# clearmatics/libff

Hardware: AMD Instinct MI355X
Metric: G1 MSM throughput (scalar-muls/sec) (higher is better)
Workload: dtype u32

## Files before the change

### libff_amd/csrc/msm_group.hip

```cpp
#include "curve_params.h"
#include "ec.cuh"
#include "fp2h.cuh"
#include "group_vtable.h"
#include "wide.cuh"
#include "wide28.cuh"
#include "rr.cuh"

#include <algorithm>
#include <cstdio>
#include <vector>
#include <type_traits>

#ifndef AMDMSM_GROUP
#error "compile with -DAMDMSM_GROUP=<group traits> -DAMDMSM_VT=<vtable getter name>"
#endif

namespace amdmsm {
template <bool I>
struct ec_coeff_a<Fp<AMDMSM_GROUP::fq, I>> {
    static constexpr int value = AMDMSM_GROUP::DEG == 1 ? AMDMSM_GROUP::COEFF_A : 0;
};
template <int NR, bool I>
struct ec_coeff_a<Fp2<AMDMSM_GROUP::fq, NR, I>> {
    static constexpr int value = AMDMSM_GROUP::DEG == 2 ? AMDMSM_GROUP::COEFF_A : 0;
// ... 1925 lines not shown
AMDMSM_DEV typename std::enable_if<(P::N >= 16 && P::N < 32), void>::type horner_chain(
    Jac<Fp<P, I>>& res, const uint32_t* __restrict__ window_sums, int W, int c, const uint32_t* __restrict__ init) {
    using F = WideFq<P>;
    const WideEnv<P> env = wide_env<P>();
    auto load = [&](const uint32_t* p, uint32_t& X, uint32_t& Y, uint32_t& Z) {
        X = env.valid ? p[env.j] : 0u;
        Y = env.valid ? p[EW + env.j] : 0u;
        Z = env.valid ? p[2 * EW + env.j] : 0u;
    };
    uint32_t X, Y, Z, X2, Y2, Z2;
    int w = W - 1;
    if (init) {
        load(init, X, Y, Z);
    } else {
        load(window_sums + (size_t)w * XYZW, X, Y, Z);
        --w;
    }
    for (; w >= 0; --w) {
        if (!wide_is_zero(Z)) {
            if (c >= 4) jac_dbl_run28<P>(env, X, Y, Z, c);
            else for (int i = 0; i < c; ++i) jac_dbl_wide2<P>(env, X, Y, Z);
        }
        load(window_sums + (size_t)w * XYZW, X2, Y2, Z2);
        jac_add_seq<F, P>(env, X, Y, Z, X2, Y2, Z2);
    }
    wide_to_packed(res.x, X);
    wide_to_packed(res.y, Y);
    wide_to_packed(res.z, Z);
}
template <class P, int NR, bool I>
AMDMSM_DEV typename std::enable_if<(P::N < 16), void>::type horner_chain(Jac<Fp2<P, NR, I>>& res,
                                                                         const uint32_t* __restrict__ window_sums, int W,
                                                                         int c, const uint32_t* __restrict__ init) {
    using F = WideFq2<P, NR>;
    const WideEnv<P> env = wide_env<P>();
    const uint32_t wi = F::word_index(env);
    auto load = [&](const uint32_t* p, uint32_t& X, uint32_t& Y, uint32_t& Z) {
        X = env.valid ? p[wi] : 0u;
        Y = env.valid ? p[EW + wi] : 0u;
        Z = env.valid ? p[2 * EW + wi] : 0u;
    };
    uint32_t X, Y, Z, X2, Y2, Z2;
    int w = W - 1;
    if (init) {
        load(init, X, Y, Z);
    } else {
        load(window_sums + (size_t)w * XYZW, X, Y, Z);
        --w;
    }
    for (; w >= 0; --w) {
        if (!wide_is_zero(Z)) {
            if constexpr (GP::COEFF_A != 0) for (int i = 0; i < c; ++i) jac_dbl_seq<F, P, GP::COEFF_A>(env, X, Y, Z);
            else if (c >= 4) jac_dbl_run28q<P, NR>(env, X, Y, Z, c);
            else for (int i = 0; i < c; ++i) jac_dbl_seq<F, P>(env, X, Y, Z);
        }
        load(window_sums + (size_t)w * XYZW, X2, Y2, Z2);
        jac_add_seq<F, P, GP::COEFF_A>(env, X, Y, Z, X2, Y2, Z2);
    }
    wide_to_packed(res.x.c0, from_row(X, 0));
    wide_to_packed(res.x.c1, from_row(X, 1));
    wide_to_packed(res.y.c0, from_row(Y, 0));
    wide_to_packed(res.y.c1, from_row(Y, 1));
    wide_to_packed(res.z.c0, from_row(Z, 0));
    wide_to_packed(res.z.c1, from_row(Z, 1));
}
template <class EE>
AMDMSM_DEV void horner_chain(Jac<EE>& res, const uint32_t* __restrict__ window_sums, int W, int c,
                             const uint32_t* __restrict__ init, ...) {
    Jac<EE> x;
    int w = W - 1;
    if (init) {
        load_jac(res, init);
    } else {
        load_jac(res, window_sums + (size_t)w * XYZW);
        --w;
    }
    for (; w >= 0; --w) {
        for (int i = 0; i < c; ++i) jac_dbl_lanes3(res);
        load_jac(x, window_sums + (size_t)w * XYZW);
        jac_add(res, res, x);
    }
}

__global__ void __launch_bounds__(64) k_horner(const uint32_t* __restrict__ window_sums, int W, int c, int form,
                                               const uint32_t* __restrict__ init, uint32_t* __restrict__ out) {
    __builtin_amdgcn_s_setprio(3);
    Jac<E> res;
    horner_chain(res, window_sums, W, c, init);
    if (threadIdx.x == 0) store_out(out, res, form);
}

constexpr int WH_MAX_GROUPS = 6;
__global__ void __launch_bounds__(64 * WH_MAX_GROUPS) k_window_horner(const uint32_t* __restrict__ planes, int c,
                                                                       uint32_t* __restrict__ out) {
    __shared__ uint32_t grp[WH_MAX_GROUPS * XYZW];
    __builtin_amdgcn_s_setprio(3);
    const int wave = (int)(threadIdx.x >> 6), ng = (c + 3) / 4;
    Jac<E> res;
    if (wave < ng) {
        const int k0 = 4 * wave, cnt = (c - k0 < 4) ? c - k0 : 4;
        horner_chain(res, planes + ((size_t)blockIdx.x * c + k0) * XYZW, cnt, 1, nullptr);
        if ((threadIdx.x & 63u) == 0) store_jac(grp + wave * XYZW, res);
    }
    __syncthreads();
    if (wave != 0) return;
    horner_chain(res, grp, ng, 4, nullptr);
    if (threadIdx.x == 0) store_jac(out + (size_t)blockIdx.x * XYZW, res);
}

struct horner_outs {
    uint32_t* p[8];
};
__global__ void __launch_bounds__(64) k_horner_batch(const uint32_t* __restrict__ window_sums, int W, int c, int form,
                                                     horner_outs outs) {
    __builtin_amdgcn_s_setprio(3);
    Jac<E> res;
    horner_chain(res, window_sums + (size_t)blockIdx.x * W * XYZW, W, c, nullptr);
    uint32_t* out = outs.p[0];
#pragma unroll
    for (int j = 1; j < 8; ++j) out = (blockIdx.x == (unsigned)j) ? outs.p[j] : out;
    if (threadIdx.x == 0) store_out(out, res, form);
}

__global__ void __launch_bounds__(64) k_sum_points(const uint32_t* __restrict__ pts, int k, int form,
                                                   uint32_t* __restrict__ out) {
    Jac<E> res;
    if (k <= 0) jac_set_inf(res);
    else horner_chain(res, pts, k, 0, nullptr);
    if (threadIdx.x == 0) store_out(out, res, form);
}

constexpr int IMPORT_K = 32;

__global__ void __launch_bounds__(TPB) k_import_bases(const uint32_t* __restrict__ src, size_t stride_words,
                                                      int form_special, size_t n, uint32_t* __restrict__ dst) {
    if (form_special) {
        const size_t i = gtid();
        if (i >= n) return;
        const uint32_t* q = src + i * stride_words;
        Aff<E> a;
        E z;
        el_load(a.x, q);
        el_load(a.y, q + EW);
        el_load(z, q + 2 * EW);
        if (el_is_zero(z)) {
            el_zero(a.x);
            el_zero(a.y);
        }
        store_aff(dst + i * AFFW, a);
        return;
    }
    const size_t i0 = gtid() * IMPORT_K;
    if (i0 >= n) return;
    const size_t i1 = (i0 + IMPORT_K < n) ? i0 + IMPORT_K : n;
    E one, acc;
    el_one(one);
    acc = one;
    bool trivial = true;
    for (size_t i = i0; i < i1; ++i) {
        Jac<E> p;
        load_libff(p, src + i * stride_words);
        if (jac_is_inf(p)) continue;
        el_store(dst + i * AFFW, acc);
        if (!el_eq(p.z, one)) {
            trivial = false;
            el_mul(acc, acc, p.z);
        }
    }
    E inv = one;
    if (!trivial) el_inv(inv, acc);
    for (size_t i = i1; i-- > i0;) {
        Jac<E> p;
        load_libff(p, src + i * stride_words);
        Aff<E> a;
        if (jac_is_inf(p)) {
            el_zero(a.x);
            el_zero(a.y);
        } else if (el_eq(p.z, one)) {
            a.x = p.x;
            a.y = p.y;
        } else {
            E pre, zi, z2;
            el_load(pre, dst + i * AFFW);
            el_mul(zi, inv, pre);
            el_mul(inv, inv, p.z);
            el_sqr(z2, zi);
            el_mul(a.x, p.x, z2);
            el_mul(z2, z2, zi);
            el_mul(a.y, p.y, z2);
        }
        store_aff(dst + i * AFFW, a);
    }
}

__global__ void __launch_bounds__(TPB) k_export_affine(const uint32_t* __restrict__ src, size_t n,
                                                       uint32_t* __restrict__ dst) {
    const size_t i = gtid();
    if (i >= n) return;
    Aff<E> a;
    load_aff(a, src + i * AFFW);
// ... 884 lines not shown
#pragma unroll
        for (int j = FRW - 1; j >= 0; --j) rec[j] = (rec[j] << SMV_W) | (j ? rec[j - 1] >> (32 - SMV_W) : 0u);
        const bool neg = (f >> (SMV_W - 1)) != 0;
        const uint32_t mag = neg ? (1u << SMV_W) - f : f;
        if (mag) {
            load_aff(e, table + ((size_t)(mag - 1) * n + i) * AFFW);
            el_cneg(e.y, e.y, neg);
            xyzz_madd(acc, e);
        }
    }
    Jac<E> res;
    xyzz_to_jac(res, acc);
    store_out(out + i * XYZW, res, form);
}

constexpr int SEG_DS = (SMV_DIGITS + 3) / 4 * 4;

__global__ void __launch_bounds__(TPB) k_seg_digits(const uint32_t* __restrict__ scalars, size_t n, int mont,
                                                    uint32_t* __restrict__ digits) {
    const size_t i = gtid();
    if (i >= n) return;
    uint32_t s[FRW];
    load_scalar(s, scalars, i, mont);
    uint32_t* row = digits + i * (SEG_DS / 4);
    uint32_t word = 0;
    for_each_signed_digit(s, SMV_W, SMV_DIGITS, [&](int w, int32_t d) {
        word |= ((uint32_t)d & 0xffu) << ((w & 3) * 8);
        if ((w & 3) == 3 || w == SMV_DIGITS - 1) {
            row[w >> 2] = word;
            word = 0;
        }
    });
}

__global__ void __launch_bounds__(TPB) k_seg_accumulate(const uint32_t* __restrict__ table, size_t nt,
                                                        const signed char* __restrict__ digits,
                                                        const uint4* __restrict__ slices, size_t lanes,
                                                        uint32_t* __restrict__ sums) {
    const size_t lane = gtid();
    if (lane >= lanes) return;
    const size_t sl = lane / SMV_DIGITS;
    const uint32_t w = (uint32_t)(lane - sl * SMV_DIGITS);
    const uint4 s = slices[sl];
    Xyzz<E> acc;
    xyzz_set_inf(acc);
    Aff<E> e;
    const signed char* dp = digits + (size_t)s.x * SEG_DS + w;
    size_t col = s.z;
#pragma unroll 1
    for (uint32_t t = s.x; t < s.y; ++t, ++col, dp += SEG_DS) {
        const int d = *dp;
        if (d) {
            const uint32_t mag = (uint32_t)(d < 0 ? -d : d);
            load_aff(e, table + ((size_t)(mag - 1) * nt + col) * AFFW);
            el_cneg(e.y, e.y, d < 0);
            xyzz_madd(acc, e);
        }
    }
    store_xyzz(sums + lane * ZZW, acc);
}

__global__ void __launch_bounds__(TPB) k_seg_fold(const uint32_t* __restrict__ sums, const uint32_t* __restrict__ seg_first,
                                                  size_t lanes, uint32_t* __restrict__ winsum) {
    const size_t lane = gtid();
    if (lane >= lanes) return;
    const size_t seg = lane / SMV_DIGITS;
    const uint32_t w = (uint32_t)(lane - seg * SMV_DIGITS);
    Xyzz<E> acc, x;
    xyzz_set_inf(acc);
#pragma unroll 1
    for (uint32_t sl = seg_first[seg]; sl < seg_first[seg + 1]; ++sl) {
        load_xyzz(x, sums + ((size_t)sl * SMV_DIGITS + w) * ZZW);
        xyzz_add(acc, acc, x);
    }
    Jac<E> r;
    xyzz_to_jac(r, acc);
    store_jac(winsum + lane * XYZW, r);
}

__global__ void __launch_bounds__(64) k_seg_horner(const uint32_t* __restrict__ winsum, int form, uint32_t* __restrict__ out) {
    Jac<E> res;
    horner_chain(res, winsum + (size_t)blockIdx.x * SMV_DIGITS * XYZW, SMV_DIGITS, SMV_W, nullptr);
    if (threadIdx.x == 0) store_out(out + (size_t)blockIdx.x * XYZW, res, form);
}

constexpr int FOLD_DS = (SMV_DIGITS + 3) / 4 * 4;
static_assert(2 * FOLD_MAX_K * FOLD_DS <= (int)FOLD_DIGIT_BYTES, "the digit rows fit the buffer the engine sets aside");
struct alignas(16) fold_scalars {
    uint32_t w[FOLD_MAX_K * FRW];
};

__global__ void __launch_bounds__(64) k_fold_digits(const fold_scalars sc, int k, int mont, int glv, int W,
                                                    uint32_t* __restrict__ digits) {
    const int j = (int)threadIdx.x;
    if (j >= k) return;
    uint32_t s[FRW];
    load_scalar(s, sc.w, (size_t)j, mont);
    uint32_t word = 0;
    auto put = [&](int row, int w, int32_t d) {
        word |= ((uint32_t)d & 0xffu) << ((w & 3) * 8);
        if ((w & 3) == 3 || w == W - 1) {
            digits[row * (FOLD_DS / 4) + (w >> 2)] = word;
            word = 0;
        }
    };
    if (glv) {
        if constexpr (GP::HAS_ENDO) for_each_glv_digit(s, SMV_W, W, [&](int h, int w, int32_t d) { put(2 * j + h, w, d); });
    } else {
        for_each_signed_digit(s, SMV_W, W, [&](int w, int32_t d) { put(j, w, d); });
    }
}

__global__ void __launch_bounds__(TPB) k_fold_ladder(const uint32_t* __restrict__ tables, size_t n,
                                                     const uint32_t* __restrict__ digits, int rows, int glv, int W,
                                                     int form, uint32_t* __restrict__ out) {
    const size_t i = gtid();
    if (i >= n) return;
    int top = -1;
#pragma unroll 1
    for (int q = (W + 3) / 4 - 1; q >= 0 && top < 0; --q) {
        uint32_t any = 0;
#pragma unroll 1
        for (int r = 0; r < rows; ++r) any |= digits[r * (FOLD_DS / 4) + q];
        if (any) top = 4 * q + (31 - __clz((int)any)) / 8;
    }
    const signed char* dg = (const signed char*)digits;
    Xyzz<E> acc;
    xyzz_set_inf(acc);
    Aff<E> e;
#pragma unroll 1
    for (int w = top; w >= 0; --w) {
        if (w != top) {
#pragma unroll 1
            for (int b = 0; b < SMV_W; ++b) xyzz_dbl(acc, acc);
        }
#pragma unroll 1
        for (int r = 0; r < rows; ++r) {
            const int d = dg[r * FOLD_DS + w];
            if (d) {
                const uint32_t mag = (uint32_t)(d < 0 ? -d : d);
                const size_t t = (size_t)(glv ? r >> 1 : r);
                load_aff(e, tables + ((t * SMV_T + (mag - 1)) * n + i) * AFFW);
                if constexpr (GP::HAS_ENDO) {
                    if (glv && (r & 1)) scale_by_beta(e.x);
                }
                el_cneg(e.y, e.y, d < 0);
                xyzz_madd(acc, e);
            }
        }
    }
    Jac<E> res;
    xyzz_to_jac(res, acc);
    store_out(out + i * XYZW, res, form);
}

inline unsigned blocks_for(size_t n, int tpb = TPB) { return (unsigned)((n + tpb - 1) / tpb); }

void l_import_bases(hipStream_t st, const uint32_t* src, size_t stride_words, int form_special, size_t n, uint32_t* dst) {
    if (!n) return;
    const size_t lanes = form_special ? n : (n + IMPORT_K - 1) / IMPORT_K;
    hipLaunchKernelGGL(k_import_bases, dim3(blocks_for(lanes)), dim3(TPB), 0, st, src, stride_words, form_special, n, dst);
}
void l_precompute_table(hipStream_t st, const uint32_t* bases, size_t n, int c, int D, uint32_t* tmp, uint32_t* table) {
    if (!n) return;
    hipLaunchKernelGGL(k_precompute_table, dim3(blocks_for(n)), dim3(TPB), 0, st, bases, n, c, D, tmp, table);
}
// ... 179 lines not shown
                fwrite(h.data(), 8, h.size(), f);
                fclose(f);
            }
        }
    }
#else
    hipLaunchKernelGGL(k_accumulate, dim3(blocks_for((size_t)W * T * ACC_LANES)), dim3(TPB), dyn_lds, st, ends, lists,
                       list_stride, bases, buckets, part_first, part_last, cont_bucket, W, B, S, T, endo_pts,
                       endo_pts ? (uint32_t)n_real : 0x80000000u, sync_waves);
#endif
}
void l_endo_points(hipStream_t st, const uint32_t* bases, size_t n, uint32_t* out) {
    if (!n) return;
    hipLaunchKernelGGL(k_endo_points, dim3(blocks_for(n * 2 * GP::DEG)), dim3(TPB), 0, st, bases, n, out);
}
void l_glv_digits(hipStream_t st, const uint32_t* scalars, size_t n, int mont, int c, int W, int32_t* out) {
    if (!n) return;
    hipLaunchKernelGGL(k_glv_digits, dim3(blocks_for(n)), dim3(TPB), 0, st, scalars, n, mont, c, W, out);
}
size_t l_accumulate_resident_lanes(int overlap) {
    auto query = [](size_t dyn_lds) {
        int dev = 0, cus = 256, blocks = 0;
        if (hipGetDevice(&dev) == hipSuccess) (void)hipDeviceGetAttribute(&cus, hipDeviceAttributeMultiprocessorCount, dev);
        if (hipOccupancyMaxActiveBlocksPerMultiprocessor(&blocks, k_accumulate, TPB, dyn_lds) != hipSuccess || blocks <= 0) blocks = 4;
        return (size_t)cus * (size_t)blocks * TPB / ACC_LANES;
    };
    static const size_t lanes = query(0);
    static const size_t lanes_overlap = (AMDMSM_OVERLAP_OK && ACC_OVERLAP_LDS) ? query(ACC_OVERLAP_LDS) : lanes;
    return overlap ? lanes_overlap : lanes;
}
void l_accumulate_fixup(hipStream_t st, const uint32_t* ends, uint32_t* buckets, uint32_t* part_first,
                        const uint32_t* part_last, const uint32_t* cont_bucket, uint32_t* queue, int W, uint32_t B,
                        uint32_t S, uint32_t T) {
    const unsigned fix_blocks = blocks_for((size_t)W * T * RED_LANES, 64);
    const unsigned compact_blocks = T / FIX_BLOCK >= 2 ? (unsigned)(W * (T / FIX_BLOCK - 1)) : 0u;
    hipLaunchKernelGGL(k_accumulate_fixup, dim3(fix_blocks + compact_blocks), dim3(64), 0, st, ends, part_first,
                       part_last, cont_bucket, buckets, queue, W, B, S, T, fix_blocks);
    const size_t lanes = (size_t)W * T;
    const size_t cap_mid = fixup_queue_cap_mid(lanes) / (RED_FOLD / MID_G) + 1, cap_long = fixup_queue_cap_long(lanes);
    const unsigned mid_blocks = (unsigned)(cap_mid < 8192 ? cap_mid : 8192), long_blocks = (unsigned)(cap_long < 2048 ? cap_long : 2048);
    hipLaunchKernelGGL(k_accumulate_fixup_queue, dim3(mid_blocks + long_blocks), dim3(64), 0, st, ends,
                       part_first, part_last, cont_bucket, buckets, queue, mid_blocks, lanes, B, S, T);
}
void l_reduce_segments(hipStream_t st, const uint32_t* buckets, int W, uint32_t B, uint32_t L, uint32_t* out) {
    hipLaunchKernelGGL(k_reduce_segments, dim3(blocks_for((size_t)W * (B / L) * RED_LANES, 64)), dim3(64), 0, st, buckets, W, B,
                       L, out);
}
void l_sum_butterfly(hipStream_t st, const uint32_t* in, int W, uint32_t M, uint32_t* out) {
    hipLaunchKernelGGL(k_sum_butterfly, dim3(blocks_for((size_t)W * M * RED_LANES, 64)), dim3(64), 0, st, in, W, M, out);
}
void l_sum_block(hipStream_t st, const uint32_t* in, int W, uint32_t M, uint32_t* out) {
    if (M >= 8 && M * RED_LANES <= (uint32_t)SUMW_THREADS && (M & (M - 1)) == 0) {
        hipLaunchKernelGGL(k_sum_block_wide, dim3(W), dim3(SUMW_THREADS), 0, st, in, W, M, out);
        return;
    }
    const unsigned threads = (unsigned)((M * RED_LANES + 63) / 64 * 64);
    hipLaunchKernelGGL(k_sum_block, dim3(W), dim3(threads), 0, st, in, W, M, out);
}
void l_reduce_rowcol(hipStream_t st, const uint32_t* buckets, int W, uint32_t B, int c, uint32_t q_row, uint32_t q_col,
                     uint32_t* rc, uint32_t* planes, uint32_t* out) {
    const int h = c / 2;
    const uint32_t C = 1u << h, R = B >> h;
    auto fit = [](uint32_t len, uint32_t q) {
        if (q < 1) q = 1;
        while (q & (q - 1)) q &= q - 1;
        if (q > len) q = len;
        while (len / q > RED_FOLD) q <<= 1;
        return q;
    };
    q_row = fit(C, q_row);
    q_col = fit(R, q_col);
    const size_t row_lanes = (size_t)W * (R + 1) * (C / q_row) * RED_LANES, col_lanes = (size_t)W * C * (R / q_col) * RED_LANES;
    const unsigned row_blocks = blocks_for(row_lanes, 64), col_blocks = blocks_for(col_lanes, 64);
    hipLaunchKernelGGL(k_bucket_sums, dim3(row_blocks + col_blocks), dim3(64), 0, st, buckets, W, B, h, q_row, q_col, row_blocks, rc);
    const uint32_t maxm = (C > R ? C : R) / 2;
    static const bool wide_planes = !(getenv("AMDMSM_PLANES_WIDE") && atoi(getenv("AMDMSM_PLANES_WIDE")) == 0);
    if (maxm >= 8 && wide_planes) {
        hipLaunchKernelGGL(k_plane_sums_wide, dim3((unsigned)(W * c)), dim3(SUMW_THREADS), 0, st, rc, W, c, h, planes);
    } else {
        unsigned threads = (unsigned)((maxm * RED_LANES + 63) / 64 * 64);
        threads = threads < 64 ? 64 : (threads > 256 ? 256 : threads);
        hipLaunchKernelGGL(k_plane_sums, dim3((unsigned)(W * c)), dim3(threads), 0, st, rc, W, c, h, planes);
    }
    hipLaunchKernelGGL(k_window_horner, dim3((unsigned)W), dim3((unsigned)(64 * ((c + 3) / 4))), 0, st, planes, c, out);
}
void l_horner(hipStream_t st, const uint32_t* window_sums, int W, int c, int form, const uint32_t* init, uint32_t* out) {
    hipLaunchKernelGGL(k_horner, dim3(1), dim3(64), 0, st, window_sums, W, c, form, init, out);
}
void l_horner_batch(hipStream_t st, const uint32_t* window_sums, int k, int W, int c, int form, uint32_t* const* outs) {
    horner_outs o = {};
    for (int j = 0; j < k && j < 8; ++j) o.p[j] = outs[j];
    hipLaunchKernelGGL(k_horner_batch, dim3((unsigned)k), dim3(64), 0, st, window_sums, W, c, form, o);
}
void l_sum_points(hipStream_t st, const uint32_t* pts, int k, int form, uint32_t* out) {
    hipLaunchKernelGGL(k_sum_points, dim3(1), dim3(64), 0, st, pts, k, form, out);
}
void l_gen_bases_seq(hipStream_t st, unsigned long long first, size_t n, uint32_t* dst) {
    if (!n) return;
    hipLaunchKernelGGL(k_gen_bases_seq, dim3(blocks_for(n)), dim3(TPB), 0, st, first, n, dst);
}
void l_export_affine(hipStream_t st, const uint32_t* src, size_t n, uint32_t* dst) {
    if (!n) return;
    hipLaunchKernelGGL(k_export_affine, dim3(blocks_for(n)), dim3(TPB), 0, st, src, n, dst);
}
void l_ffi_decode_points(hipStream_t st, const uint32_t* src, size_t n, uint32_t* dst, uint32_t* status) {
    if (!n) return;
    hipLaunchKernelGGL(k_ffi_decode_points, dim3(blocks_for(n)), dim3(TPB), 0, st, src, n, dst, status);
}
void l_ffi_decode_scalars(hipStream_t st, const uint32_t* src, size_t n, uint32_t* dst, uint32_t* status) {
    if (!n) return;
    hipLaunchKernelGGL(k_ffi_decode_scalars, dim3(blocks_for(n)), dim3(TPB), 0, st, src, n, dst, status);
}
void l_ffi_encode_point(hipStream_t st, const uint32_t* src_xyz, uint32_t* dst) {
    hipLaunchKernelGGL(k_ffi_encode_point, dim3(1), dim3(64), 0, st, src_xyz, dst);
}
void l_disk_decode(hipStream_t st, const uint32_t* src, size_t n, uint32_t* dst) {
    if (!n) return;
    hipLaunchKernelGGL(k_disk_decode, dim3(blocks_for(n)), dim3(TPB), 0, st, src, n, dst);
}
void l_disk_decode_compressed(hipStream_t st, const uint32_t* src, size_t n, uint32_t* dst, uint32_t* status) {
    if (!n) return;
    hipLaunchKernelGGL(k_disk_decode_compressed, dim3(blocks_for(n, 64)), dim3(64), 0, st, src, n, dst, status);
}
#if AMDMSM_ACC_RR
template <class G>
bool launch_fb_exp_rr(hipStream_t st, const uint32_t* table_aff, const uint32_t* scalars, size_t n, int mont, const uint32_t* coeff,
                      int scalar_size, int window, int form, uint32_t* out) {
    if constexpr (G::DEG == 1) {
        if (window < 32) {
            hipLaunchKernelGGL(k_fb_exp_rr<G>, dim3(blocks_for(n)), dim3(TPB), 0, st, table_aff, scalars, n, mont, coeff, scalar_size,
                               window, form, out);
            return true;
        }
    }
    return false;
}
#endif
void l_fixed_base_exp(hipStream_t st, const uint32_t* g_xyz, int scalar_size, int window, const uint32_t* scalars, size_t n,
                      int mont, const uint32_t* coeff, int form, uint32_t* gouter, uint32_t* table, uint32_t* table_aff,
                      int build_table, uint32_t* out) {
    const int outerc = (scalar_size + window - 1) / window;
    if (build_table) {
        hipLaunchKernelGGL(k_fb_gouter, dim3(1), dim3(64), 0, st, g_xyz, outerc, window, gouter);
        for (int level = 0; level < window; ++level) {
            const size_t per_level = level == 0 ? 2 : ((size_t)1 << level);
            hipLaunchKernelGGL(k_fb_table_level, dim3(blocks_for((size_t)outerc * per_level)), dim3(TPB), 0, st, gouter, outerc,
                               window, scalar_size, level, table);
        }
        const size_t entries = (size_t)outerc << window;
        hipLaunchKernelGGL(k_fb_table_affine, dim3(blocks_for((entries + FB_NORM_K - 1) / FB_NORM_K)), dim3(TPB), 0, st, table,
                           entries, table_aff);
    }
    if (n) {
#if AMDMSM_ACC_RR
        if (launch_fb_exp_rr<GP>(st, table_aff, scalars, n, mont, coeff, scalar_size, window, form, out)) return;
#endif
        hipLaunchKernelGGL(k_fb_exp, dim3(blocks_for(n)), dim3(TPB), 0, st, table_aff, scalars, n, mont, coeff, scalar_size,
                           window, form, out);
    }
}
void l_field_op(hipStream_t st, int op, const uint32_t* a, const uint32_t* b, uint32_t* out, size_t n) {
    if (!n) return;
    hipLaunchKernelGGL(k_field_op, dim3(blocks_for(n)), dim3(TPB), 0, st, op, a, b, out, n);
}
void l_field_probe(hipStream_t st, int impl, int op, const uint32_t* a, const uint32_t* b, const uint32_t* c, const uint32_t* d,
                   uint32_t* out, uint32_t* flag, size_t n) {
    if (!n) return;
    if (impl) hipLaunchKernelGGL(k_field_probe<EI>, dim3(blocks_for(n)), dim3(TPB), 0, st, op, a, b, c, d, out, flag, n);
    else hipLaunchKernelGGL(k_field_probe<E>, dim3(blocks_for(n)), dim3(TPB), 0, st, op, a, b, c, d, out, flag, n);
}
void l_xyzz_probe(hipStream_t st, int impl, int op, const uint32_t* acc, const uint32_t* pt, uint32_t* out, size_t n) {
    if (!n) return;
    if (impl) hipLaunchKernelGGL(k_xyzz_probe<EI>, dim3(blocks_for(n)), dim3(TPB), 0, st, op, acc, pt, out, n);
    else hipLaunchKernelGGL(k_xyzz_probe<E>, dim3(blocks_for(n)), dim3(TPB), 0, st, op, acc, pt, out, n);
}
void l_group_op(hipStream_t st, int op, const uint32_t* a, const uint32_t* b, uint32_t* out, size_t n, int form) {
    if (!n) return;
    hipLaunchKernelGGL(k_group_op, dim3(blocks_for(n)), dim3(TPB), 0, st, op, a, b, out, n, form);
}
void l_digits(hipStream_t st, const uint32_t* scalars, size_t n, int mont, int c, int W, int32_t* out) {
    if (!n) return;
    hipLaunchKernelGGL(k_digits, dim3(blocks_for(n)), dim3(TPB), 0, st, scalars, n, mont, c, W, out);
}
void l_mul_bench(hipStream_t st, uint32_t* inout, size_t nthreads, int iters, int inline_variant) {
    if (!nthreads) return;
#if AMDMSM_BENCH_BOTH
    if (inline_variant) {
        hipLaunchKernelGGL(k_mul_bench<true>, dim3(blocks_for(nthreads)), dim3(TPB), 0, st, inout, nthreads, iters);
        return;
    }
#endif
    hipLaunchKernelGGL(k_mul_bench<false>, dim3(blocks_for(nthreads)), dim3(TPB), 0, st, inout, nthreads, iters);
}
void l_madd_bench(hipStream_t st, const uint32_t* pts, uint32_t* out, size_t nthreads, int iters, int inline_variant) {
    if (!nthreads) return;
    if (inline_variant == 2) {
        hipLaunchKernelGGL(k_xyzz_madd_bench<EH>, dim3(blocks_for(nthreads)), dim3(TPB), 0, st, pts, out, nthreads, iters);
        return;
    }
#if AMDMSM_BENCH_BOTH
    if (inline_variant) {
        hipLaunchKernelGGL(k_madd_bench<EI>, dim3(blocks_for(nthreads)), dim3(TPB), 0, st, pts, out, nthreads, iters);
        return;
    }
#endif
    hipLaunchKernelGGL(k_madd_bench<E>, dim3(blocks_for(nthreads)), dim3(TPB), 0, st, pts, out, nthreads, iters);
}
void l_smv_table(hipStream_t st, const uint32_t* bases, size_t n, uint32_t* tmp, uint32_t* table) {
    if (!n) return;
    hipLaunchKernelGGL(k_smv_table, dim3(blocks_for(n)), dim3(TPB), 0, st, bases, n, tmp, table);
}
void l_smv_ladder(hipStream_t st, const uint32_t* table, size_t n, const uint32_t* scalars, int mont, int form, uint32_t* out) {
    if (!n) return;
    hipLaunchKernelGGL(k_smv_ladder, dim3(blocks_for(n)), dim3(TPB), 0, st, table, n, scalars, mont, form, out);
}
void l_seg_digits(hipStream_t st, const uint32_t* scalars, size_t n, int mont, uint32_t* digits) {
    if (!n) return;
    hipLaunchKernelGGL(k_seg_digits, dim3(blocks_for(n)), dim3(TPB), 0, st, scalars, n, mont, digits);
}
void l_seg_accumulate(hipStream_t st, const uint32_t* table, size_t nt, const uint32_t* digits, const uint32_t* slices,
                      size_t n_slices, uint32_t* sums) {
    if (!n_slices) return;
    const size_t lanes = n_slices * SMV_DIGITS;
    hipLaunchKernelGGL(k_seg_accumulate, dim3(blocks_for(lanes)), dim3(TPB), 0, st, table, nt, (const signed char*)digits,
                       (const uint4*)slices, lanes, sums);
}
void l_seg_fold(hipStream_t st, const uint32_t* sums, const uint32_t* seg_first, size_t m, uint32_t* winsum) {
    if (!m) return;
    const size_t lanes = m * SMV_DIGITS;
    hipLaunchKernelGGL(k_seg_fold, dim3(blocks_for(lanes)), dim3(TPB), 0, st, sums, seg_first, lanes, winsum);
}
void l_seg_horner(hipStream_t st, const uint32_t* winsum, size_t m, int form, uint32_t* out) {
    if (!m) return;
    hipLaunchKernelGGL(k_seg_horner, dim3((unsigned)m), dim3(64), 0, st, winsum, form, out);
}
void l_fold_digits(hipStream_t st, const uint32_t* scalars_host, int k, int mont, int glv, int W, uint32_t* digits) {
    if (k < 1 || k > FOLD_MAX_K) return;
    fold_scalars sc = {};
    std::copy(scalars_host, scalars_host + (size_t)k * FRW, sc.w);
    hipLaunchKernelGGL(k_fold_digits, dim3(1), dim3(64), 0, st, sc, k, mont, GP::HAS_ENDO ? glv : 0, W, digits);
}
void l_fold_ladder(hipStream_t st, const uint32_t* tables, size_t n, const uint32_t* digits, int rows, int glv, int W, int form,
                   uint32_t* out) {
    if (!n) return;
    hipLaunchKernelGGL(k_fold_ladder, dim3(blocks_for(n)), dim3(TPB), 0, st, tables, n, digits, rows, GP::HAS_ENDO ? glv : 0, W,
                       form, out);
}

const group_vtable g_vt = {
    GP::CURVE, GP::GROUP, FRW, EW, FQ::N, FR::BITS, GP::LIBFF_PROJECTIVE ? 1 : 0, (int)RED_FOLD, ZZS, FR::R,
    GLV::BOUND_LOG2_X1000, GP::SUBGROUP_CHECK == 0 ? 1 : 0, GLV::LAMBDA, l_endo_points, l_glv_digits,
    l_import_bases, l_precompute_table, l_count, l_scatter, l_scalar_stats, l_sort, l_accumulate, l_accumulate_resident_lanes, (AMDMSM_OVERLAP_OK && ACC_OVERLAP_LDS) ? 1 : 0, l_accumulate_fixup, l_reduce_segments, l_sum_butterfly, l_sum_block, l_reduce_rowcol, l_horner, l_horner_batch, l_sum_points,
    l_gen_bases_seq, l_export_affine, l_ffi_decode_points, l_ffi_decode_scalars, l_ffi_encode_point, l_disk_decode, l_disk_decode_compressed, l_fixed_base_exp, l_field_op, l_group_op, l_digits, l_mul_bench, l_madd_bench,
    GP::HAS_ENDO ? 1 : 0, GP::COEFF_A != 0 ? 1 : 0, l_sort_sel, l_gather_scalars, l_scalar_bits, l_sort_short,
    SMV_T, l_smv_table, l_smv_ladder,
    SMV_DIGITS, SEG_DS, l_seg_digits, l_seg_accumulate, l_seg_fold, l_seg_horner,
    l_field_probe, l_xyzz_probe,
    l_sort_top_window,
    FOLD_DS, l_fold_digits, l_fold_ladder,
};

}

const group_vtable* AMDMSM_VT() { return &g_vt; }

}
```

### libff_amd/csrc/wide28.cuh

```cuda
#pragma once
#include "wide.cuh"

namespace amdmsm {

template <int NW>
struct cbig {
    uint32_t w[NW];
};
template <int NW>
constexpr bool cb_ge(const cbig<NW>& a, const cbig<NW>& b) {
    for (int i = NW - 1; i >= 0; --i) {
        if (a.w[i] != b.w[i]) return a.w[i] > b.w[i];
    }
    return true;
}
template <int NW>
constexpr cbig<NW> cb_sub(const cbig<NW>& a, const cbig<NW>& b) {
    cbig<NW> r{};
    uint64_t borrow = 0;
    for (int i = 0; i < NW; ++i) {
        const uint64_t d = (uint64_t)a.w[i] - b.w[i] - borrow;
        r.w[i] = (uint32_t)d;
        borrow = (d >> 32) & 1u;
    }
// ... 141 lines not shown

template <class P>
AMDMSM_DEV void jac_dbl_28(const Env28<P, 10>& v, uint32_t& X, uint32_t& Y, uint32_t& Z) {
    const uint32_t row = (threadIdx.x & 63u) >> 4;
    uint32_t r = mul28(v, row == 0 ? X : Y, row == 0 ? X : (row == 1 ? Y : Z));
    const uint32_t XX = from_row(r, 0), B = from_row(r, 1), YZ = from_row(r, 2);
    const uint32_t B2 = B + B, E3 = XX + XX + XX;
    r = mul28(v, row == 0 ? B2 : (row == 1 ? X : E3), row == 2 ? E3 : B2);
    const uint32_t C4 = from_row(r, 0), XB2 = from_row(r, 1), F = from_row(r, 2);
    const uint32_t D = XB2 + XB2;
    X = sub28_16(v, F, D + D);
    const uint32_t t = mul28(v, E3, sub28_32(v, D, X));
    Y = sub28_16(v, t, C4 + C4);
    Z = YZ + YZ;
}

template <class P, int HEAD>
AMDMSM_DEV uint32_t to28(const Env28<P, HEAD>& v, uint32_t w) {
    constexpr uint32_t RM = (uint32_t)WideEnv<P>::ROW - 1u;
    const uint32_t rowbase = threadIdx.x & 63u & ~RM;
    const uint32_t bit = 28u * v.j, q = bit >> 5, o = bit & 31u;
    const uint32_t lo = (uint32_t)__shfl((int)w, (int)(rowbase + (q & RM)), 64);
    const uint32_t hi = (uint32_t)__shfl((int)w, (int)(rowbase + ((q + 1) & RM)), 64);
    const uint64_t both = ((uint64_t)hi << 32) | lo;
    const uint32_t limb = v.j < (uint32_t)W28<P, HEAD>::L ? (uint32_t)(both >> o) & MASK28 : 0u;
    return mul28(v, limb, v.cin);
}
template <class P, int HEAD>
AMDMSM_DEV uint32_t from28(const Env28<P, HEAD>& v, uint32_t a) {
    const uint32_t r = mul28(v, a, v.cout);
    const uint32_t s = (r & MASK28) + row_up1<P>(v.e, r >> 28);
    const unsigned long long cin = carry_in_mask((s >> 28) != 0u, s == MASK28);
    const uint32_t n = (s + (__builtin_amdgcn_inverse_ballot_w64(cin) ? 1u : 0u)) & MASK28;
    constexpr uint32_t RM = (uint32_t)WideEnv<P>::ROW - 1u;
    const uint32_t rowbase = threadIdx.x & 63u & ~RM;
    const uint32_t bit = 32u * v.j, q = bit / 28u, o = bit % 28u;
    const uint32_t l0 = (uint32_t)__shfl((int)n, (int)(rowbase + (q & RM)), 64);
    const uint32_t l1 = (uint32_t)__shfl((int)n, (int)(rowbase + ((q + 1) & RM)), 64);
    const uint32_t word = v.e.valid ? (l0 >> o) | (uint32_t)((uint64_t)l1 << (28u - o)) : 0u;
    return wide_cond_sub_p<P>(v.e, word);
}

template <class P>
AMDMSM_DEV void jac_dbl_28_two(const Env28<P, 10>& v, uint32_t& X, uint32_t& Y, uint32_t& Z) {
    const bool r1 = (threadIdx.x & 32u) != 0;
    uint32_t r = mul28(v, r1 ? Y : X, r1 ? Y : X);
    const uint32_t XX = row_copy<P>(v.e, r, 0), B = row_copy<P>(v.e, r, 1);
    const uint32_t B2 = B + B, E3 = XX + XX + XX;
    r = mul28(v, r1 ? B2 : Y, r1 ? B2 : Z);
    const uint32_t YZ = row_copy<P>(v.e, r, 0), C4 = row_copy<P>(v.e, r, 1);
    r = mul28(v, r1 ? E3 : X, r1 ? E3 : B2);
    const uint32_t XB2 = row_copy<P>(v.e, r, 0), F = row_copy<P>(v.e, r, 1);
    const uint32_t D = XB2 + XB2;
    X = sub28_16(v, F, D + D);
    const uint32_t t = mul28(v, E3, sub28_32(v, D, X));
    Y = sub28_16(v, t, C4 + C4);
    Z = YZ + YZ;
}

template <class P>
AMDMSM_DEV void jac_dbl_run28(const WideEnv<P>& e, uint32_t& X, uint32_t& Y, uint32_t& Z, int c) {
    const Env28<P, 10> v = env28<P, 10>(e);
    if constexpr (WideEnv<P>::ROW == 16) {
        const uint32_t row = (threadIdx.x & 63u) >> 4;
        uint32_t r = to28(v, row == 0 ? X : (row == 1 ? Y : Z));
        uint32_t X28 = from_row(r, 0), Y28 = from_row(r, 1), Z28 = from_row(r, 2);
        for (int i = 0; i < c; ++i) jac_dbl_28<P>(v, X28, Y28, Z28);
        r = from28(v, row == 0 ? X28 : (row == 1 ? Y28 : carry28(v, Z28)));
        X = from_row(r, 0);
        Y = from_row(r, 1);
        Z = from_row(r, 2);
    } else {
        const bool r1 = (threadIdx.x & 32u) != 0;
        uint32_t r = to28(v, r1 ? Y : X);
        uint32_t X28 = row_copy<P>(e, r, 0), Y28 = row_copy<P>(e, r, 1), Z28 = to28(v, Z);
        for (int i = 0; i < c; ++i) jac_dbl_28_two<P>(v, X28, Y28, Z28);
        r = from28(v, r1 ? Y28 : X28);
        X = row_copy<P>(e, r, 0);
        Y = row_copy<P>(e, r, 1);
        Z = from28(v, carry28(v, Z28));
    }
}

template <class P, int NR>
struct WideFq2_28 {
    static constexpr int HEAD = 20;
    using V = Env28<P, HEAD>;
    static AMDMSM_DEV uint32_t mul(const V& v, uint32_t a, uint32_t b) {
        const uint32_t row = (threadIdx.x & 63u) >> 4;
        const bool r2 = row == 2, odd = (row & 1u) != 0;
        const uint32_t sa = a + row_swap(a), sb = b + row_swap(b);
        const uint32_t r = mul28(v, r2 ? sa : a, r2 ? sb : b);
        const uint32_t v0 = from_row(r, 0), v1 = from_row(r, 1), v2 = from_row(r, 2);
        const uint32_t nv1 = NR == -1 ? v1 : (v1 << 2) + v1;
        return carry28(v, (odd ? v2 : v0) + v.q16 - (odd ? v0 + v1 : nv1));
    }
    static AMDMSM_DEV uint32_t sqr(const V& v, uint32_t a) {
        if constexpr (NR != -1) {
            return mul(v, a, a);
        } else {
            const uint32_t row = (threadIdx.x & 63u) >> 4;
            const uint32_t sw = row_swap(a);
            const uint32_t s = a + sw, d = carry28(v, a + v.q512 - sw);
            const uint32_t r = mul28(v, row == 2 ? s : a, row == 2 ? d : sw);
            const uint32_t c0 = from_row(r, 2), x = from_row(r, 0);
            return (row & 1u) ? x + x : c0;
        }
    }
};
template <class P, int NR>
AMDMSM_DEV void jac_dbl_28q(const Env28<P, 20>& v, uint32_t& X, uint32_t& Y, uint32_t& Z) {
    using F = WideFq2_28<P, NR>;
    const uint32_t XX = F::sqr(v, X), B = F::sqr(v, Y), YZ = F::mul(v, Y, Z);
    const uint32_t B2 = carry28(v, B + B), E3 = carry28(v, XX + XX + XX);
    const uint32_t C4 = F::sqr(v, B2), XB2 = F::mul(v, X, B2);
    const uint32_t C8 = carry28(v, C4 + C4), D = carry28(v, XB2 + XB2);
    X = carry28(v, F::sqr(v, E3) + v.q128 - carry28(v, D + D));
    const uint32_t t = F::mul(v, E3, carry28(v, D + v.q256 - X));
    Y = carry28(v, t + v.q64 - C8);
    Z = carry28(v, YZ + YZ);
}
template <class P, int NR>
AMDMSM_DEV void jac_dbl_run28q(const WideEnv<P>& e, uint32_t& X, uint32_t& Y, uint32_t& Z, int c) {
    const Env28<P, 20> v = env28<P, 20>(e);
    uint32_t X28 = to28(v, X), Y28 = to28(v, Y), Z28 = to28(v, Z);
    for (int i = 0; i < c; ++i) jac_dbl_28q<P, NR>(v, X28, Y28, Z28);
    X = from28(v, X28);
    Y = from28(v, Y28);
    Z = from28(v, Z28);
}

}
```

Baseline: 642.2 million.

## Run Horner window combination in lazy 28-bit limb form end to end

Adds a Horner chain that keeps the running point in the 28-bit redundant-limb representation across all doublings and additions. It uses a new jac_add_28 with exact zero checks and converts back to packed form only at the end. This removes the repeated conversions and full reductions of the packed-field Horner path. The new path is enabled by default for degree-1, a=0 curves and can be turned off with an environment variable. It adds code complexity and depends on headroom assertions holding for correctness.

```diff
diff --git a/libff_amd/csrc/msm_group.hip b/libff_amd/csrc/msm_group.hip
--- a/libff_amd/csrc/msm_group.hip
+++ b/libff_amd/csrc/msm_group.hip
@@ -2031,11 +2031,56 @@
     }
 }
 
+constexpr bool HORNER_LAZY_OK = GP::DEG == 1 && FQ::N < 16 && GP::COEFF_A == 0;
+template <class P, bool I>
+AMDMSM_DEV void horner_chain_lazy(Jac<Fp<P, I>>& res, const uint32_t* __restrict__ window_sums, int W, int c,
+                                  const uint32_t* __restrict__ init) {
+    const WideEnv<P> env = wide_env<P>();
+    const Env28<P, 10> v = env28<P, 10>(env);
+    const uint32_t sub4 = tab28_sel(A28<P>::SUB4, env.j);
+    const uint32_t row = (threadIdx.x & 63u) >> 4;
+    auto load = [&](const uint32_t* p, uint32_t& X, uint32_t& Y, uint32_t& Z) {
+        const uint32_t r = to28(v, (env.valid && row < 3u) ? p[row * EW + env.j] : 0u);
+        X = from_row(r, 0);
+        Y = from_row(r, 1);
+        Z = from_row(r, 2);
+    };
+    uint32_t X, Y, Z, X2, Y2, Z2;
+    int w = W - 1;
+    if (init) {
+        load(init, X, Y, Z);
+    } else {
+        load(window_sums + (size_t)w * XYZW, X, Y, Z);
+        --w;
+    }
+    for (; w >= 0; --w) {
+        load(window_sums + (size_t)w * XYZW, X2, Y2, Z2);
+        if (!wide_is_zero(Z)) for (int i = 0; i < c; ++i) jac_dbl_28<P>(v, X, Y, Z);
+        jac_add_28<P>(v, sub4, X, Y, Z, X2, Y2, Z2);
+    }
+    const uint32_t r = from28(v, row == 0 ? X : (row == 1 ? Y : Z));
+    wide_to_packed(res.x, from_row(r, 0));
+    wide_to_packed(res.y, from_row(r, 1));
+    wide_to_packed(res.z, from_row(r, 2));
+}
+inline bool horner_lazy() {
+    static const bool on = HORNER_LAZY_OK && !(getenv("AMDMSM_HORNER_LAZY") && atoi(getenv("AMDMSM_HORNER_LAZY")) == 0);
+    return on;
+}
+
 __global__ void __launch_bounds__(64) k_horner(const uint32_t* __restrict__ window_sums, int W, int c, int form,
                                                const uint32_t* __restrict__ init, uint32_t* __restrict__ out) {
     __builtin_amdgcn_s_setprio(3);
     Jac<E> res;
     horner_chain(res, window_sums, W, c, init);
+    if (threadIdx.x == 0) store_out(out, res, form);
+}
+template <class EE = E>
+__global__ void __launch_bounds__(64) k_horner_lazy(const uint32_t* __restrict__ window_sums, int W, int c, int form,
+                                                    const uint32_t* __restrict__ init, uint32_t* __restrict__ out) {
+    __builtin_amdgcn_s_setprio(3);
+    Jac<EE> res;
+    horner_chain_lazy(res, window_sums, W, c, init);
     if (threadIdx.x == 0) store_out(out, res, form);
 }
 
@@ -2056,6 +2101,23 @@
     horner_chain(res, grp, ng, 4, nullptr);
     if (threadIdx.x == 0) store_jac(out + (size_t)blockIdx.x * XYZW, res);
 }
+template <class EE = E>
+__global__ void __launch_bounds__(64 * WH_MAX_GROUPS) k_window_horner_lazy(const uint32_t* __restrict__ planes, int c,
+                                                                            uint32_t* __restrict__ out) {
+    __shared__ uint32_t grp[WH_MAX_GROUPS * XYZW];
+    __builtin_amdgcn_s_setprio(3);
+    const int wave = (int)(threadIdx.x >> 6), ng = (c + 3) / 4;
+    Jac<EE> res;
+    if (wave < ng) {
+        const int k0 = 4 * wave, cnt = (c - k0 < 4) ? c - k0 : 4;
+        horner_chain_lazy(res, planes + ((size_t)blockIdx.x * c + k0) * XYZW, cnt, 1, nullptr);
+        if ((threadIdx.x & 63u) == 0) store_jac(grp + wave * XYZW, res);
+    }
+    __syncthreads();
+    if (wave != 0) return;
+    horner_chain_lazy(res, grp, ng, 4, nullptr);
+    if (threadIdx.x == 0) store_jac(out + (size_t)blockIdx.x * XYZW, res);
+}
 
 struct horner_outs {
     uint32_t* p[8];
@@ -2065,6 +2127,17 @@
     __builtin_amdgcn_s_setprio(3);
     Jac<E> res;
     horner_chain(res, window_sums + (size_t)blockIdx.x * W * XYZW, W, c, nullptr);
+    uint32_t* out = outs.p[0];
+#pragma unroll
+    for (int j = 1; j < 8; ++j) out = (blockIdx.x == (unsigned)j) ? outs.p[j] : out;
+    if (threadIdx.x == 0) store_out(out, res, form);
+}
+template <class EE = E>
+__global__ void __launch_bounds__(64) k_horner_batch_lazy(const uint32_t* __restrict__ window_sums, int W, int c, int form,
+                                                          horner_outs outs) {
+    __builtin_amdgcn_s_setprio(3);
+    Jac<EE> res;
+    horner_chain_lazy(res, window_sums + (size_t)blockIdx.x * W * XYZW, W, c, nullptr);
     uint32_t* out = outs.p[0];
 #pragma unroll
     for (int j = 1; j < 8; ++j) out = (blockIdx.x == (unsigned)j) ? outs.p[j] : out;
@@ -3115,6 +3188,55 @@
     Jac<E> res;
     horner_chain(res, winsum + (size_t)blockIdx.x * SMV_DIGITS * XYZW, SMV_DIGITS, SMV_W, nullptr);
     if (threadIdx.x == 0) store_out(out + (size_t)blockIdx.x * XYZW, res, form);
+}
+template <class EE = E>
+__global__ void __launch_bounds__(64) k_seg_horner_lazy(const uint32_t* __restrict__ winsum, int form, uint32_t* __restrict__ out) {
+    Jac<EE> res;
+    horner_chain_lazy(res, winsum + (size_t)blockIdx.x * SMV_DIGITS * XYZW, SMV_DIGITS, SMV_W, nullptr);
+    if (threadIdx.x == 0) store_out(out + (size_t)blockIdx.x * XYZW, res, form);
+}
+
+template <bool OK> struct horner_lazy_el { using type = E; };
+template <bool OK = HORNER_LAZY_OK>
+void launch_horner(hipStream_t st, const uint32_t* window_sums, int W, int c, int form, const uint32_t* init, uint32_t* out) {
+    if constexpr (OK) {
+        if (horner_lazy()) {
+            hipLaunchKernelGGL(k_horner_lazy<typename horner_lazy_el<OK>::type>, dim3(1), dim3(64), 0, st, window_sums, W, c, form, init, out);
+            return;
+        }
+    }
+    hipLaunchKernelGGL(k_horner, dim3(1), dim3(64), 0, st, window_sums, W, c, form, init, out);
+}
+template <bool OK = HORNER_LAZY_OK>
+void launch_horner_batch(hipStream_t st, const uint32_t* window_sums, int k, int W, int c, int form, const horner_outs& o) {
+    if constexpr (OK) {
+        if (horner_lazy()) {
+            hipLaunchKernelGGL(k_horner_batch_lazy<typename horner_lazy_el<OK>::type>, dim3((unsigned)k), dim3(64), 0, st, window_sums, W, c, form, o);
+            return;
+        }
+    }
+    hipLaunchKernelGGL(k_horner_batch, dim3((unsigned)k), dim3(64), 0, st, window_sums, W, c, form, o);
+}
+template <bool OK = HORNER_LAZY_OK>
+void launch_window_horner(hipStream_t st, const uint32_t* planes, int W, int c, uint32_t* out) {
+    const dim3 threads((unsigned)(64 * ((c + 3) / 4)));
+    if constexpr (OK) {
+        if (horner_lazy()) {
+            hipLaunchKernelGGL(k_window_horner_lazy<typename horner_lazy_el<OK>::type>, dim3((unsigned)W), threads, 0, st, planes, c, out);
+            return;
+        }
+    }
+    hipLaunchKernelGGL(k_window_horner, dim3((unsigned)W), threads, 0, st, planes, c, out);
+}
+template <bool OK = HORNER_LAZY_OK>
+void launch_seg_horner(hipStream_t st, const uint32_t* winsum, size_t m, int form, uint32_t* out) {
+    if constexpr (OK) {
+        if (horner_lazy()) {
+            hipLaunchKernelGGL(k_seg_horner_lazy<typename horner_lazy_el<OK>::type>, dim3((unsigned)m), dim3(64), 0, st, winsum, form, out);
+            return;
+        }
+    }
+    hipLaunchKernelGGL(k_seg_horner, dim3((unsigned)m), dim3(64), 0, st, winsum, form, out);
 }
 
 constexpr int FOLD_DS = (SMV_DIGITS + 3) / 4 * 4;
@@ -3460,15 +3582,15 @@
         threads = threads < 64 ? 64 : (threads > 256 ? 256 : threads);
         hipLaunchKernelGGL(k_plane_sums, dim3((unsigned)(W * c)), dim3(threads), 0, st, rc, W, c, h, planes);
     }
-    hipLaunchKernelGGL(k_window_horner, dim3((unsigned)W), dim3((unsigned)(64 * ((c + 3) / 4))), 0, st, planes, c, out);
+    launch_window_horner(st, planes, W, c, out);
 }
 void l_horner(hipStream_t st, const uint32_t* window_sums, int W, int c, int form, const uint32_t* init, uint32_t* out) {
-    hipLaunchKernelGGL(k_horner, dim3(1), dim3(64), 0, st, window_sums, W, c, form, init, out);
+    launch_horner(st, window_sums, W, c, form, init, out);
 }
 void l_horner_batch(hipStream_t st, const uint32_t* window_sums, int k, int W, int c, int form, uint32_t* const* outs) {
     horner_outs o = {};
     for (int j = 0; j < k && j < 8; ++j) o.p[j] = outs[j];
-    hipLaunchKernelGGL(k_horner_batch, dim3((unsigned)k), dim3(64), 0, st, window_sums, W, c, form, o);
+    launch_horner_batch(st, window_sums, k, W, c, form, o);
 }
 void l_sum_points(hipStream_t st, const uint32_t* pts, int k, int form, uint32_t* out) {
     hipLaunchKernelGGL(k_sum_points, dim3(1), dim3(64), 0, st, pts, k, form, out);
@@ -3610,7 +3732,7 @@
 }
 void l_seg_horner(hipStream_t st, const uint32_t* winsum, size_t m, int form, uint32_t* out) {
     if (!m) return;
-    hipLaunchKernelGGL(k_seg_horner, dim3((unsigned)m), dim3(64), 0, st, winsum, form, out);
+    launch_seg_horner(st, winsum, m, form, out);
 }
 void l_fold_digits(hipStream_t st, const uint32_t* scalars_host, int k, int mont, int glv, int W, uint32_t* digits) {
     if (k < 1 || k > FOLD_MAX_K) return;
diff --git a/libff_amd/csrc/wide28.cuh b/libff_amd/csrc/wide28.cuh
--- a/libff_amd/csrc/wide28.cuh
+++ b/libff_amd/csrc/wide28.cuh
@@ -247,6 +247,80 @@
     }
 }
 
+template <class P>
+struct A28 {
+    using T = W28<P, 10>;
+    static constexpr tab28 SUB4 = T::lifted(2, 30);
+    static constexpr uint32_t PTOP = cb_limb28(T::modulus(), T::J, true) + 1;
+    static_assert(SUB4.v[T::J] >= PTOP * 2 && T::SUB16.v[T::J] >= PTOP * 8 && T::SUB32.v[T::J] >= PTOP * 18, "top-limb headroom");
+    static_assert((1u << 30) - 4u >= 3u * ((1u << 28) + (1u << 5)), "lift covers a three-term subtrahend");
+    static_assert((uint64_t)(1u << 28) + (1u << 5) + (1u << 30) + (1u << 28) < (1ull << 32), "lifted difference fits a lane");
+    static constexpr uint64_t OP = 872000000ull;
+    static_assert(3ull * ((1u << 28) + (1u << 5)) < OP && 2ull * ((1u << 28) + (1u << 5)) + (1u << 6) < OP, "operand limbs");
+    static_assert(OP * OP + (1ull << 56) + (1ull << 32) < (1ull << 63), "64-bit column");
+    static_assert(((OP * OP + (1ull << 56) + (1ull << 32)) >> 28) + (1ull << 28) < (1ull << 32), "shifted column");
+    static_assert(28 * T::L >= P::BITS + 10 && T::L < 16, "headroom of the radix; lane 15 of a row stays empty");
+};
+
+template <class P>
+AMDMSM_DEV void exact28(const Env28<P, 10>& v, uint32_t r, unsigned long long& nz, unsigned long long& np) {
+    const uint32_t s = (r & MASK28) + row_up1<P>(v.e, r >> 28);
+    const unsigned long long cin = carry_in_mask((s >> 28) != 0u, s == MASK28);
+    const uint32_t n = (s + (__builtin_amdgcn_inverse_ballot_w64(cin) ? 1u : 0u)) & MASK28;
+    nz = __ballot(n != 0u);
+    np = __ballot(n != v.pj);
+}
+template <int ROW>
+AMDMSM_DEV bool row_zero28(unsigned long long nz, unsigned long long np) {
+    return ((nz >> (16 * ROW)) & 0xffffull) == 0ull || ((np >> (16 * ROW)) & 0xffffull) == 0ull;
+}
+
+template <class P>
+AMDMSM_DEV void jac_add_28(const Env28<P, 10>& v, uint32_t sub4, uint32_t& X1, uint32_t& Y1, uint32_t& Z1, uint32_t X2,
+                           uint32_t Y2, uint32_t Z2) {
+    const uint32_t row = (threadIdx.x & 63u) >> 4;
+    const bool r0 = row == 0, r1 = row == 1, r2 = row == 2;
+    unsigned long long nz, np;
+    uint32_t r = mul28(v, r1 ? Z2 : Z1, r0 ? Z1 : Z2);
+    exact28(v, r, nz, np);
+    const bool inf1 = row_zero28<0>(nz, np), inf2 = row_zero28<1>(nz, np);
+    if (inf2) {
+        if (inf1) Z1 = 0u;
+        return;
+    }
+    if (inf1) {
+        X1 = X2;
+        Y1 = Y2;
+        Z1 = Z2;
+        return;
+    }
+    const uint32_t z1z1 = from_row(r, 0), z2z2 = from_row(r, 1), z1z2 = from_row(r, 2);
+    r = mul28(v, r0 ? X1 : (r1 ? X2 : (r2 ? Z2 : Z1)), (r0 || r2) ? z2z2 : z1z1);
+    const uint32_t u1 = from_row(r, 0), u2 = from_row(r, 1), t1 = from_row(r, 2), t2 = from_row(r, 3);
+    const uint32_t h = carry28(v, u2 + sub4 - u1), h2 = h + h;
+    r = mul28(v, r0 ? Y1 : (r1 ? Y2 : (r2 ? h2 : z1z2)), r0 ? t1 : (r1 ? t2 : (r2 ? h2 : h)));
+    exact28(v, r, nz, np);
+    const bool hzero = row_zero28<2>(nz, np);
+    const uint32_t s1 = from_row(r, 0), s2 = from_row(r, 1), ii = from_row(r, 2), zh = from_row(r, 3);
+    const uint32_t d = carry28(v, s2 + sub4 - s1), rr = d + d;
+    if (hzero) {
+        exact28(v, mul28(v, rr, v.cout), nz, np);
+        if (row_zero28<0>(nz, np)) {
+            jac_dbl_28<P>(v, X1, Y1, Z1);
+            exact28(v, mul28(v, Z1, v.cout), nz, np);
+            if (row_zero28<0>(nz, np)) Z1 = 0u;
+            return;
+        }
+    }
+    r = mul28(v, r0 ? h : (r1 ? u1 : rr), r2 ? rr : ii);
+    const uint32_t J = from_row(r, 0), V = from_row(r, 1), R2 = from_row(r, 2);
+    X1 = sub28_16(v, R2, J + V + V);
+    r = mul28(v, r0 ? rr : s1, r0 ? sub28_32(v, V, X1) : J);
+    const uint32_t sj = from_row(r, 1);
+    Y1 = sub28_16(v, from_row(r, 0), sj + sj);
+    Z1 = hzero ? 0u : zh + zh;
+}
+
 template <class P, int NR>
 struct WideFq2_28 {
     static constexpr int HEAD = 20;
```

Result: faster. 649.7 million (median of 6 runs) (+1.2%).
